# qcraftai/gedepth

Measured on AMD Instinct MI355X. Metric: training img/s (whole node), KITTI-shaped 352x1120 synthetic batches, higher is better.
Workload: dtype bf16; 1 GPU; depthformer_swint_v: DepthFormer-SwinT + GEDepth-Vanilla, 352x1120, 8 img/GPU, full train step; global_batch=8, parallelism=dp1, allreduce_dtype=fp32, layout=nhwc, window_attention=bf16 mfma, params=53516992, hip_graph=off

## Files before the change

gedepth_amd/csrc/common.h:

```cpp
#pragma once
#include <hip/hip_runtime.h>
#include <stdint.h>
#include "../../include/gedepth_hip.h"

#define GE_WAVE 64

#define GE_LAUNCH_CHECK()                         \
  do {                                            \
    hipError_t e__ = hipGetLastError();           \
    if (e__ != hipSuccess) return (int)e__;       \
  } while (0)

typedef uint16_t bf16_t;

__device__ __forceinline__ float bf2f(bf16_t h) { return __uint_as_float(((uint32_t)h) << 16); }
typedef __bf16 ge_bf16x8 __attribute__((ext_vector_type(8)));
typedef __bf16 ge_bf16x4 __attribute__((ext_vector_type(4)));
typedef __bf16 ge_bf16x2 __attribute__((ext_vector_type(2)));
typedef float ge_f32x16 __attribute__((ext_vector_type(16)));
typedef unsigned int ge_u32x4 __attribute__((ext_vector_type(4)));
typedef short ge_s16x2 __attribute__((ext_vector_type(2)));
#define GE_LDS(T, p) ((__attribute__((address_space(3))) T*)(p))

__device__ __forceinline__ bf16_t f2bf_hw(float f) { return __builtin_bit_cast(bf16_t, (__bf16)f); }
__device__ __forceinline__ uint32_t ge_pack_bf16x2(float lo, float hi) {
  ge_bf16x2 v = {(__bf16)lo, (__bf16)hi};
  return __builtin_bit_cast(uint32_t, v);
}
__device__ __forceinline__ bf16_t f2bf(float f) {
#ifndef GE_SW_BF16
  return f2bf_hw(f);
#endif
  uint32_t u = __float_as_uint(f);
  if ((u & 0x7fffffffu) > 0x7f800000u) return (bf16_t)((u >> 16) | 0x40u);
  u += 0x7fffu + ((u >> 16) & 1u);
  return (bf16_t)(u >> 16);
}

template <typename T> struct Io;
template <> struct Io<float> {
  static __device__ __forceinline__ float ld(const float* p) { return *p; }
  static __device__ __forceinline__ void st(float* p, float v) { *p = v; }
  static __device__ __forceinline__ float rt(float v) { return v; }
};
template <> struct Io<bf16_t> {
  static __device__ __forceinline__ float ld(const bf16_t* p) { return bf2f(*p); }
  static __device__ __forceinline__ void st(bf16_t* p, float v) { *p = f2bf(v); }
  static __device__ __forceinline__ float rt(float v) { return bf2f(f2bf(v)); }
};

template <typename T, int N> struct Vec;
template <> struct Vec<float, 4> {
  static __device__ __forceinline__ void ld(const float* p, float v[4]) { const float4 t = *(const float4*)p; v[0] = t.x; v[1] = t.y; v[2] = t.z; v[3] = t.w; }
  static __device__ __forceinline__ void st(float* p, const float v[4]) { *(float4*)p = make_float4(v[0], v[1], v[2], v[3]); }
};
template <> struct Vec<float, 8> {
  static __device__ __forceinline__ void ld(const float* p, float v[8]) { Vec<float, 4>::ld(p, v); Vec<float, 4>::ld(p + 4, v + 4); }
  static __device__ __forceinline__ void st(float* p, const float v[8]) { Vec<float, 4>::st(p, v); Vec<float, 4>::st(p + 4, v + 4); }
};
// ... 149 lines not shown
```

gedepth_amd/csrc/nhwc.hip:

```cpp
#include "common.h"
#include "../../include/gedepth_neck.h"

#define NH_MAXLANES 256

#define NH_MAXBLOCKS 1024
template <int K, int VN>
__device__ __forceinline__ void nh_col_commit(float (&acc)[K][VN], float* __restrict__ partial, int C, int lpr, int rpi, int c0) {
  __shared__ float sm[K][NH_MAXLANES][VN];
  const int t = threadIdx.x, rs = t / lpr;
#pragma unroll
  for (int k = 0; k < K; ++k)
#pragma unroll
    for (int v = 0; v < VN; ++v) sm[k][t][v] = acc[k][v];
  __syncthreads();
  int span = 1;
  while (span < rpi) span <<= 1;
  for (int stride = span >> 1; stride > 0; stride >>= 1) {
    if (rs < stride && rs + stride < rpi) {
#pragma unroll
      for (int k = 0; k < K; ++k)
#pragma unroll
        for (int v = 0; v < VN; ++v) sm[k][t][v] += sm[k][t + stride * lpr][v];
    }
    __syncthreads();
// ... 682 lines not shown
static int colsum_launch(const void* x, long R, int C, float* out, void* ws, int accumulate, hipStream_t s) {
  constexpr int VN = V8<T>::N;
  if (C % VN || !nh_aligned(x)) return GE_ERR_UNSUPPORTED;
  const int lanes = C / VN;
  int lpr = lanes < NH_MAXLANES ? lanes : NH_MAXLANES;
  while (lanes % lpr) --lpr;
  const int rpi = NH_MAXLANES / lpr, chunks = lanes / lpr;
  unsigned gx = nh_grid_rows(R, rpi);
  if (chunks > 1) gx = (gx + chunks - 1) / chunks;
  if (!gx) gx = 1;
  colsum_k<T><<<dim3(gx, chunks), 256, 0, s>>>((const T*)x, nh_partials(ws, C, 1), C, R, lpr, rpi);
  GE_LAUNCH_CHECK();
  nh_reduce_launch_f32(ws, C, gx, out, accumulate, s);
  GE_LAUNCH_CHECK();
  return GE_OK;
}
extern "C" int ge_colsum(const void* x, long R, int C, float* out, void* workspace, int accumulate, int dtype, void* stream) {
  if (!x || !out || !workspace || R < 0 || C <= 0) return GE_ERR_BAD_ARG;
  if (dtype == GE_F32) return colsum_launch<float>(x, R, C, out, workspace, accumulate, ge_stream(stream));
  if (dtype == GE_BF16) return colsum_launch<bf16_t>(x, R, C, out, workspace, accumulate, ge_stream(stream));
  return GE_ERR_UNSUPPORTED;
}

struct NhLevels { int s[GE_NECK_MAX_LEVELS + 1]; };
struct NhParts { const void* p[GE_NECK_MAX_LEVELS]; long pitch[GE_NECK_MAX_LEVELS]; long col[GE_NECK_MAX_LEVELS]; };
static bool nh_levels(const long* starts, int n, long N, NhLevels& lv, long& longest) {
  if (!starts || n < 1 || n > GE_NECK_MAX_LEVELS || N <= 0 || N > NH_WALK_MAX_ROWS || starts[0] != 0 || starts[n] != N) return false;
  longest = 0;
  for (int l = 0; l <= GE_NECK_MAX_LEVELS; ++l) lv.s[l] = (int)N;
  for (int l = 0; l < n; ++l) {
    if (starts[l + 1] < starts[l]) return false;
    lv.s[l] = (int)starts[l];
    if (starts[l + 1] - starts[l] > longest) longest = starts[l + 1] - starts[l];
  }
  return true;
}

template <typename T>
__global__ void __launch_bounds__(256) add_rows_levels_k(const T* __restrict__ x, const float* __restrict__ pos, const float* __restrict__ emb,
                                                         T* __restrict__ out, int B, long N, int C, NhLevels lv, int lpr, int rpi) {
  constexpr int VN = V8<T>::N;
  const int t = threadIdx.x, lane = t % lpr, rs = t / lpr, level = blockIdx.y;
  const int start = lv.s[level], nl = lv.s[level + 1] - start;
  if (rs >= rpi || nl <= 0) return;
  const int c0 = lane * VN;
  float e[VN];
// ... 247 lines not shown
```

gedepth_amd/depth/models/necks/hahi.py:

```python
import os

import torch
import torch.nn as nn
import torch.nn.functional as F

from .... import kernels as K
from .... import neck_kernels as NK
from ....kernels import add_rows, concat_tokens_map, ms_deform_attn_raw, residual_dropout, tokens_from_map
from ....mmrt import bricks
from ....mmrt.bricks import BaseModule, ConvModule, build_positional_encoding, xavier_init
from ..builder import ATTENTION, NECKS


@ATTENTION.register_module()
class MultiScaleDeformableAttention(BaseModule):

    def __init__(self, embed_dims=256, num_heads=8, num_levels=4, num_points=4, im2col_step=64, dropout=0.1,
                 batch_first=False, norm_cfg=None, init_cfg=None):
        super().__init__(init_cfg)
        if embed_dims % num_heads != 0:
            raise ValueError(f'embed_dims must be divisible by num_heads, but got {embed_dims} and {num_heads}')
        if embed_dims // num_heads != 64:
            raise NotImplementedError('the HIP sampling kernel is specialised for 64 channels per head')
        self.norm_cfg, self.batch_first = norm_cfg, batch_first
        self.dropout = nn.Dropout(dropout)
        self.im2col_step = im2col_step
        self.embed_dims, self.num_levels, self.num_heads, self.num_points = embed_dims, num_levels, num_heads, num_points
        self.sampling_offsets = nn.Linear(embed_dims, num_heads * num_levels * num_points * 2)
        self.attention_weights = nn.Linear(embed_dims, num_heads * num_levels * num_points)
        self.value_proj = bricks.Linear(embed_dims, embed_dims)
        self.output_proj = bricks.Linear(embed_dims, embed_dims)
        self.init_weights()

    def init_weights(self):
        bricks.constant_init(self.sampling_offsets, 0.)
        self.sampling_offsets.bias.data = bricks.msda_offset_bias(self.num_heads, self.num_levels, self.num_points)
        bricks.constant_init(self.attention_weights, val=0., bias=0.)
        xavier_init(self.value_proj, distribution='uniform', bias=0.)
        xavier_init(self.output_proj, distribution='uniform', bias=0.)
        self._is_init = True

    def _attend(self, query, value, reference_points, spatial_shapes, key_padding_mask=None, query_shapes=None, query_order=None):
        bs, num_query, _ = query.shape
        num_value = value.shape[1]
        if torch.is_tensor(spatial_shapes):
            spatial_shapes = [(int(h), int(w)) for h, w in spatial_shapes.tolist()]
        assert sum(h * w for h, w in spatial_shapes) == num_value
        if reference_points.shape[-1] != 2:
            raise ValueError('only 2-d reference points are used on the GEDepth path')
        value = self.value_proj(value)
        if key_padding_mask is not None:
            value = value.masked_fill(key_padding_mask[..., None], 0.0)
        value = value.view(bs, num_value, self.num_heads, -1)
        nH, L, P = self.num_heads, self.num_levels, self.num_points
        w = torch.cat((self.sampling_offsets.weight, self.attention_weights.weight), 0)
        b = torch.cat((self.sampling_offsets.bias, self.attention_weights.bias), 0)
        raw = bricks.linear_tokens(query, w, b)
        if raw.dtype != value.dtype:
            raw = raw.to(value.dtype)
        ref = reference_points.expand(bs, num_query, L, 2)
        if query_order is not None and 'msda_mm' not in K.DISABLED and K.msda_mm_supported(value, raw, spatial_shapes, nH, L, P):
            out = K.ms_deform_attn_mm(value, raw, ref, spatial_shapes, query_order, nH, L, P)
        elif K.msda_self_split_ok(value, raw, spatial_shapes, query_shapes, nH, L, P):
            out = K.ms_deform_attn_self_split(value, raw, ref, spatial_shapes, nH, L, P)
        else:
            out = ms_deform_attn_raw(value, raw, ref, spatial_shapes, query_shapes, nH, L, P)
        return self.output_proj(out)

    def forward(self, query, key=None, value=None, identity=None, query_pos=None, key_padding_mask=None,
                reference_points=None, spatial_shapes=None, level_start_index=None, query_shapes=None, query_order=None, **kwargs):
        if value is None:
            value = query
        if identity is None:
            identity = query
        if query_pos is not None:
            if query_pos.dim() == 3 and query_pos.shape[0] == 1 and query_pos.dtype == torch.float32 and query.dim() == 3 and self.batch_first:
                query = add_rows(query, query_pos[0])
            else:
                query = query + query_pos.to(query.dtype)
        if not self.batch_first:
            query, value = query.permute(1, 0, 2), value.permute(1, 0, 2)
        out = self._attend(query, value, reference_points, spatial_shapes, key_padding_mask, query_shapes, query_order)
        if not self.batch_first:
            out = out.permute(1, 0, 2)
        if self.training and self.dropout.p > 0 and out.is_cuda and out.dim() == 3 and self.batch_first:
            return residual_dropout(identity, out, self.dropout.p)
        return self.dropout(out) + identity

    def forward_map(self, fmap, pos_map, value, reference_points, spatial_shapes, concat_with, query_order=None, query=None):
        if query is None:
            query = tokens_from_map(fmap, pos_map)
        out = self._attend(query, value, reference_points, spatial_shapes, query_shapes=[tuple(fmap.shape[2:])], query_order=query_order)
        p = self.dropout.p if self.training else 0.0
        return concat_tokens_map(out, concat_with, identity=fmap, tokens_first=True, p_drop=p)


@NECKS.register_module()
class HAHIHeteroNeck(BaseModule):

    def __init__(self, in_channels, out_channels, embedding_dim, scales=[1, 1, 1, 1],
                 norm_cfg=dict(type='BN', requires_grad=True), act_cfg=dict(type='ReLU', inplace=True),
                 cross_att=True, self_att=True, constrain=False, positional_encoding=None, num_points=8):
        super().__init__()
        assert isinstance(in_channels, list)
        assert all(s == 1 for s in scales), 'GEDepth configs use scale 1 at every level'
        self.cross_att, self.self_att, self.constrain = cross_att, self_att, constrain
        self.in_channels, self.out_channels, self.scales = in_channels, out_channels, scales
        self.num_outs = len(scales)
        self.embedding_dim = E = embedding_dim
        cm = dict(norm_cfg=norm_cfg, act_cfg=act_cfg)
        self.lateral_convs = nn.ModuleList(ConvModule(i, o, kernel_size=1, **cm) for i, o in zip(in_channels, out_channels))
        self.trans_proj = nn.ModuleList(ConvModule(o, E, kernel_size=1, **cm) for o in out_channels[1:])
        self.trans_fusion = nn.ModuleList(ConvModule(o + E, o, kernel_size=3, padding=1, stride=1, **cm)
                                          for o in out_channels[1:])
        self.conv_proj = nn.Sequential(ConvModule(in_channels[0], E, kernel_size=1, **cm))
        self.conv_fusion = nn.Sequential(ConvModule(in_channels[0] + E, out_channels[0], kernel_size=3, padding=1,
                                                    stride=1, **cm))
# ... 134 lines not shown
```

gedepth_amd/hip.py:

```python
import ctypes
import os
import re

import torch

_HERE = os.path.dirname(os.path.abspath(__file__))
LIB_PATH = os.environ.get('GE_LIB') or os.path.join(_HERE, 'csrc', 'libgedepth_hip.so')
HEADERS = {'SIGNATURES': 'gedepth_hip.h', 'EVAL_SIGNATURES': 'gedepth_eval.h', 'DDAD_SIGNATURES': 'gedepth_ddad.h',
           'CLOUD_SIGNATURES': 'gedepth_cloud.h', 'GROUND_SIGNATURES': 'gedepth_ground.h'}
EXTRA_HEADERS = {'BATCH_SIGNATURES': 'gedepth_batch.h'}
SCENE_HEADERS = {'SCENE_SIGNATURES': 'gedepth_scene.h'}
STRATA_HEADERS = {'STRATA_SIGNATURES': 'gedepth_strata.h'}
NECK_HEADERS = {'NECK_SIGNATURES': 'gedepth_neck.h'}
GE_F32, GE_BF16 = 0, 1
GE_COLORIZE_VMIN_DATA, GE_COLORIZE_VMAX_DATA, GE_COLORIZE_EQUAL = 1, 2, 4

_SCALARS = {'int': ctypes.c_int, 'long': ctypes.c_long, 'float': ctypes.c_float, 'double': ctypes.c_double, 'size_t': ctypes.c_size_t,
            'uint64_t': ctypes.c_ulonglong, 'unsigned long long': ctypes.c_ulonglong}
_DECL = re.compile(r'\b(int|size_t)\s+(ge_\w+)\s*\(([^()]*)\)\s*;')


def parse_header(text):
    text = re.sub(r'/\*.*?\*/|//[^\n]*', ' ', text, flags=re.S)
    sigs = {}
    for res, name, params in _DECL.findall(text):
        args = []
        for p in ([] if params.strip() == 'void' else params.split(',')):
            if '*' in p:
                args.append(ctypes.c_void_p)
                continue
            ctype = ' '.join(w for w in p.split()[:-1] if w != 'const')
            if ctype not in _SCALARS:
                raise TypeError(f'{name}: parameter "{" ".join(p.split())}" has a type the ctypes binding does not map')
            args.append(_SCALARS[ctype])
        sigs[name] = (_SCALARS[res], args)
    stray = set(re.findall(r'\b(ge_\w+)\s*\(', text)) - set(sigs)
    if stray:
        raise TypeError(f'cannot parse the declaration of {", ".join(sorted(stray))}')
    return sigs


for _table, _header in {**HEADERS, **EXTRA_HEADERS, **SCENE_HEADERS, **STRATA_HEADERS, **NECK_HEADERS}.items():
    with open(os.path.join(os.path.dirname(_HERE), 'include', _header)) as _fh:
        globals()[_table] = parse_header(_fh.read())

_lib = None


class HipLibraryError(RuntimeError):
    pass


def lib():
    global _lib
    if _lib is None:
        if not os.path.isfile(LIB_PATH):
            raise HipLibraryError(
                f'{LIB_PATH} is missing: the gfx950 HIP kernels are not built. '
                f'Run gedepth_amd/csrc/build.sh (hipcc --offload-arch=gfx950). There is no CPU/eager fallback.')
        handle = ctypes.CDLL(LIB_PATH)
        for table in (*HEADERS, *EXTRA_HEADERS, *SCENE_HEADERS, *STRATA_HEADERS, *NECK_HEADERS):
            for name, (res, args) in globals()[table].items():
                fn = getattr(handle, name)
                fn.restype, fn.argtypes = res, args
        _lib = handle
        if os.environ.get('GE_MSDA_MODE'):
            handle.ge_msda_mode(int(os.environ['GE_MSDA_MODE']))
    return _lib


def is_built():
    return os.path.isfile(LIB_PATH)


def check(code, what):
    if code != 0:
        raise RuntimeError(f'{what} failed with code {code} '
                           f'({"bad argument" if code == 10001 else "unsupported" if code == 10002 else "hipError_t"})')


def call(name, *args):
    code = getattr(_lib or lib(), name)(*args)
    if code:
        check(code, name)
# ... 26 lines not shown
```

gedepth_amd/kernels.py:

```python
import ctypes
import os

import torch

from . import hip

_f32 = torch.float32


def _c(t):
    return t if t.is_contiguous() else t.contiguous()


class _Profiler:

    def __init__(self):
        self.on, self.records, self.stage_bytes = False, {}, {}

    def enable(self):
        self.on, self.records, self.stage_bytes = True, {}, {}
        hip.lib().ge_msda_bwd_timing(1)

    def disable(self):
        self.on = False
# ... 256 lines not shown
    nbytes = (value.numel() * _es(value) + (loc.numel() + attw.numel()) * 4 + d_raw.numel() * es + d_out.numel() * _es(d_out)
              + (0 if d_value is None else d_value.numel() * 4))
    _launch(f'msda_bwd_raw[B{B} Nq{Nq} Nv{Nv} {_tag(value)}{" lw" if d_value is None else ""}]', nbytes, 'ge_msda_bwd_raw', hip.ptr(value), lv.ptr,
            grid.ptr, grid.n, hip.ptr(loc), hip.ptr(attw), hip.ptr(d_out), hip.ptr(d_value), base, ld, base + nH * L * P * 2 * es, ld, hip.ptr(d_ref),
            hip.ptr(ws), ws_bytes, B, Nv, Nq, nH, L, P, hip.dtype_code(value), hip.stream())
    return d_raw, d_ref


def _bwd_value_records(raw, raw_ref, d_out, d_value, lv, nH, L, P, level_mask=15):
    B, Nq, _ = raw.shape
    Nv = d_value.shape[1]
    n_off = nH * L * P * 2
    ws_bytes = int(hip.lib().ge_msda_bwd_workspace(lv.ptr, B, Nv, Nq, nH, L, P))
    ws = torch.empty(ws_bytes, device=raw.device, dtype=torch.uint8)
    frac = bin(level_mask).count('1') / 4
    if PROFILER.on:
        PROFILER.add_stage_bytes((0, B * Nq * n_off * 2, 0, raw.numel() * 2, int(frac * d_out.numel() * 2) + d_value.numel() * 4))
    _launch(f'msda_bwd_value_raw[B{B} Nq{Nq} Nv{Nv}{"" if level_mask == 15 else f" levels {level_mask:04b}"}]',
            B * Nq * n_off * 2 + raw.numel() * 2 + d_out.numel() * 2 + d_value.numel() * 4, 'ge_msda_bwd_value_raw_levels', lv.ptr,
            *raw_ref, hip.ptr(d_out), hip.ptr(d_value), hip.ptr(ws), ws_bytes, level_mask, B, Nv, Nq, nH, L, P,
            hip.dtype_code(d_out), hip.stream())


class _MSDeformAttnRaw(torch.autograd.Function):

    @staticmethod
    def forward(ctx, value, raw, ref, spatial_shapes, query_shapes, nH, L, P):
        value, raw = _c(value), _c(raw)
        assert value.shape[3] == 64 and raw.shape[2] == nH * L * P * 3 and raw.dtype == value.dtype
        lv, grid = _levels(spatial_shapes), _query_grid(query_shapes, raw.shape[1])
        out, loc, attw, ref = _window_fwd_raw(value, raw, ref, lv, grid, nH, L, P)
        ctx.value_from_raw = (value.dtype == torch.bfloat16 and L == 4 and P == 8 and 'msda_value_raw' not in DISABLED
                              and max(max(hw) for hw in lv.hw) <= 8191)
        if ctx.value_from_raw:
            ctx.save_for_backward(value, loc, attw, raw, ref)
        else:
            ctx.save_for_backward(value, loc, attw)
        ctx.meta = (lv, grid, nH, L, P)
        ctx.last_loc = loc
        return out

    @staticmethod
    def backward(ctx, d_out):
        value, loc, attw = ctx.saved_tensors[:3]
        split = ctx.value_from_raw
        lv, grid, nH, L, P = ctx.meta
        d_out = _c(d_out.to(value.dtype))
        d_value = torch.zeros(value.shape, device=value.device, dtype=_f32)
        d_raw, d_ref = _window_bwd_raw(value, loc, attw, d_out, lv, grid, None if split else d_value, ctx.needs_input_grad[2])
        if PROFILER.on:
            lw_b = value.numel() * _es(value) + (loc.numel() + attw.numel()) * 4 + d_raw.numel() * _es(d_raw) + d_out.numel() * _es(d_out)
            la_b = (loc.numel() + attw.numel()) * 4
            PROFILER.add_stage_bytes((lw_b, 0, 0, 0, 0) if split else (lw_b, la_b, 0, la_b, d_out.numel() * _es(d_out) + d_value.numel() * 4))
        if split:
            raw, ref = ctx.saved_tensors[3:]
            _bwd_value_records(raw, _raw_ref(raw, ref, nH, L, P)[0], d_out, d_value, lv, nH, L, P)
        return d_value.to(value.dtype), d_raw, d_ref, None, None, None, None, None


def ms_deform_attn_raw(value, raw, reference_points, spatial_shapes, query_shapes, num_heads, num_levels, num_points):
    B, Nv = value.shape[:2]
    Nq = raw.shape[1]
    fused = ('msda_raw' not in DISABLED and query_shapes is not None and MSDA_BINNED_BACKWARD and value.is_cuda and raw.dtype == value.dtype
             and value.dtype in (_f32, torch.bfloat16))
    if fused:
        lv, grid = _levels(spatial_shapes), _query_grid(query_shapes, Nq)
        fused = bool(hip.lib().ge_msda_raw_supported(lv.ptr, grid.ptr, grid.n, B, Nv, Nq, num_heads, num_levels, num_points))
        fused = fused and int(hip.lib().ge_msda_bwd_workspace(lv.ptr, B, Nv, Nq, num_heads, num_levels, num_points)) > 0
    if not fused:
        loc, attw = msda_prepare(raw, reference_points, spatial_shapes, num_heads, num_levels, num_points)
        return ms_deform_attn(value, spatial_shapes, loc, attw, query_shapes)
    return _MSDeformAttnRaw.apply(value, raw, reference_points, spatial_shapes, query_shapes, int(num_heads), int(num_levels), int(num_points))


_TILE_ORDER_CACHE = {}


def msda_tile_order(query_shapes, device, th=4, tw=8):
    key = (tuple(tuple(int(v) for v in hw) for hw in query_shapes), str(device), th, tw)
    if key not in _TILE_ORDER_CACHE:
        parts, start = [], 0
        for h, w in key[0]:
            idx = torch.arange(h * w, dtype=torch.int64).view(h, w)
            ph, pw = (-h) % th, (-w) % tw
            idx = torch.nn.functional.pad(idx, (0, pw, 0, ph), value=-1)
            hh, ww = idx.shape
            t = idx.view(hh // th, th, ww // tw, tw).permute(0, 2, 1, 3).reshape(-1)
            parts.append(t[t >= 0] + start)
            start += h * w
        _TILE_ORDER_CACHE[key] = torch.cat(parts).to(torch.int32).to(device)
    return _TILE_ORDER_CACHE[key]


# ... 68 lines not shown
                self.mm_mask = 15 if t_mm < (1.1 if on else 0.9) * t_rec else 0
                self.last = dict(rows=rows, passes=passes, mm_ms=round(t_mm * 1e-6, 3), records_ms=round(t_rec * 1e-6, 3),
                                 per_level=[dict(rows=int(host[2 + 2 * l]), passes=int(host[3 + 2 * l])) for l in range(4)])


_MM_VALUE_CHOICE = {}


def _mm_value_choice(key, mm_ok, rec_ok):
    c = _MM_VALUE_CHOICE.get(key)
    if c is None:
        c = _MM_VALUE_CHOICE[key] = _MMValueChoice()
    c.update()
    mask = c.mm_mask if c.forced is None else c.forced
    mask = 0 if not mm_ok else 15 if not rec_ok else mask
    return c, mask


class _MSDeformAttnMM(torch.autograd.Function):

    @staticmethod
    def forward(ctx, value, raw, ref, order, spatial_shapes, nH, L, P):
        lv = _levels(spatial_shapes)
        out = msda_fwd_mm(value, raw, ref, lv, order, want_loc=False, nH=nH, L=L, P=P)
        ctx.save_for_backward(value, raw, ref, order)
        ctx.meta = (lv, nH, L, P)
        return out

    @staticmethod
    def backward(ctx, d_out):
        value, raw, ref, order = ctx.saved_tensors
        lv, nH, L, P = ctx.meta
        value, raw = _c(value), _c(raw)
        B, Nv, _, D = value.shape
        _, Nq, ld = raw.shape
        d_out = _c(d_out.to(value.dtype))
        raw_ref, ref = _raw_ref(raw, ref, nH, L, P)
        lib = hip.lib()
        d_raw = torch.empty(B, Nq, ld, device=value.device, dtype=raw.dtype)
        dbase = hip.ptr(d_raw)
        nb_lw = value.numel() * 2 + raw.numel() * 2 + d_raw.numel() * 2 + d_out.numel() * 2
        want_dv = ctx.needs_input_grad[0]
        use_vs = (want_dv and os.environ.get('GE_MSDA_VALUE') == 'vs' and B * Nq * ld * 2 < 2 ** 32 and B * Nq * nH * D * 2 < 2 ** 32
                  and 0 <= ref.stride(1) and Nq * ref.stride(1) * 4 < 2 ** 32)
        vs_ws_bytes = int(lib.ge_msda_bwd_vs_workspace(lv.ptr, B, Nv, Nq, nH, L, P)) if use_vs else 0
        mm_ws_bytes = int(lib.ge_msda_bwd_mm_workspace(B, Nq, nH, L)) if (want_dv and 'msda_value_mm' not in DISABLED) else 0
        if vs_ws_bytes:
            mm_ws_bytes = vs_ws_bytes
        mm_ws = torch.empty(mm_ws_bytes, device=value.device, dtype=torch.uint8) if mm_ws_bytes else None
        _launch(f'msda_mm_bwd_lw_k[B{B} Nq{Nq} Nv{Nv}]', nb_lw, 'ge_msda_bwd_lw_mm', hip.ptr(value), lv.ptr, *raw_ref, hip.ptr(order), hip.ptr(d_out),
                dbase, ld, dbase + nH * L * P * 2 * 2, ld, hip.ptr(mm_ws), B, Nv, Nq, nH, L, P, hip.dtype_code(value), hip.stream())
        d_ref = None
        if ctx.needs_input_grad[2]:
            d_ref = torch.empty(B, Nq, L, 2, device=value.device, dtype=_f32)
            hip.call('ge_msda_dref', dbase, ld, lv.ptr, hip.ptr(d_ref), B * Nq, nH, L, P, hip.dtype_code(value), hip.stream())
        d_value = None
        if want_dv:
            d_value = torch.zeros(B, Nv, nH, D, device=value.device, dtype=_f32)
            if vs_ws_bytes:
                _launch(f'msda_mm_bwd_vs_k[B{B} Nq{Nq} Nv{Nv}]', raw.numel() * 2 + d_out.numel() * 2 + d_value.numel() * 4, 'ge_msda_bwd_value_vs', lv.ptr,
                        *raw_ref, hip.ptr(order), hip.ptr(d_out), hip.ptr(d_value), hip.ptr(mm_ws), mm_ws_bytes, B, Nv, Nq, nH, L, P,
                        hip.dtype_code(value), hip.stream())
                return d_value.to(value.dtype), d_raw, d_ref, None, None, None, None, None
            rec_ws_bytes = int(lib.ge_msda_bwd_workspace(lv.ptr, B, Nv, Nq, nH, L, P))
            choice, mm_mask = _mm_value_choice((B, Nq, Nv, nH, lv.hw, str(value.device)), mm_ws is not None, rec_ws_bytes > 0)
            rec_mask = 15 & ~mm_mask

            def value_mm(dv, mask):
                return (lv.ptr, *raw_ref, hip.ptr(order), hip.ptr(d_out), hip.ptr(dv), hip.ptr(mm_ws), mm_ws_bytes, mask, B, Nv, Nq, nH, L, P,
                        hip.dtype_code(value), hip.stream())
            if mm_mask:
                lv_rows = sum(h * w for l, (h, w) in enumerate(lv.hw) if (mm_mask >> l) & 1)
                _launch(f'msda_mm_bwd_v_k[B{B} Nq{Nq} Nv{Nv} levels {mm_mask:04b}]',
                        bin(mm_mask).count('1') * (raw.numel() // 2 + d_out.numel() * 2 // 4) + B * lv_rows * nH * D * 4, 'ge_msda_bwd_value_mm',
                        *value_mm(d_value, mm_mask))
            elif mm_ws is not None and choice.wants_stats():
                hip.call('ge_msda_bwd_value_mm', *value_mm(None, 0))
            if rec_mask:
                if rec_ws_bytes <= 0:
                    raise RuntimeError('ms_deform_attn_mm backward: neither the MFMA d_value kernel nor the binned path covers this geometry')
                _bwd_value_records(raw, raw_ref, d_out, d_value, lv, nH, L, P, rec_mask)
            if mm_ws is not None:
                choice.observe(mm_ws, int(lib.ge_msda_bwd_mm_stats_offset(B, Nq, nH, L)), B * Nq * nH)
            d_value = d_value.to(value.dtype)
        return d_value, d_raw, d_ref, None, None, None, None, None


def msda_mm_supported(value, raw, spatial_shapes, nH, L, P):
    if not (value.is_cuda and value.dtype == torch.bfloat16 and raw.dtype == torch.bfloat16 and value.shape[-1] == 64):
        return False
    B, Nv = value.shape[:2]
    return bool(hip.lib().ge_msda_mm_supported(_levels(spatial_shapes).ptr, B, Nv, raw.shape[1], nH, L, P, hip.GE_BF16))


def ms_deform_attn_mm(value, raw, reference_points, spatial_shapes, order, num_heads=8, num_levels=4, num_points=8):
    return _MSDeformAttnMM.apply(value, raw, reference_points, order, spatial_shapes, int(num_heads), int(num_levels), int(num_points))


class _MSDeformAttnSelfSplit(torch.autograd.Function):

    @staticmethod
    def forward(ctx, value, raw, ref, spatial_shapes, n_fine, order_fine, nH, L, P):
        value, raw = _c(value), _c(raw)
        B, Nv, _, D = value.shape
        _, Nq, ld = raw.shape
        assert D == 64 and ld == nH * L * P * 3 and raw.dtype == value.dtype == torch.bfloat16 and 0 < n_fine < Nq
        raw_ref, ref = _raw_ref(raw, ref, nH, L, P)
        lv = _levels(spatial_shapes)
        out = torch.empty(B, Nq, nH * D, device=value.device, dtype=value.dtype)
        nc = Nq - n_fine
        _launch(f'msda_mm_fwd_k[B{B} Nq{n_fine}/{Nq} Nv{Nv}]', value.numel() * 2 + B * n_fine * (ld + nH * D) * 2, 'ge_msda_fwd_mm_part',
                hip.ptr(value, name='value'), lv.ptr, *raw_ref, hip.ptr(order_fine), hip.ptr(out), B, Nv, n_fine, Nq, nH, L, P, hip.GE_BF16, hip.stream())
        coarse_shapes = []
        acc = 0
        for hw in lv.hw:
            acc += hw[0] * hw[1]
            if acc > n_fine:
                coarse_shapes.append(hw)
        assert sum(h * w for h, w in coarse_shapes) == nc, 'n_fine must end on a level boundary'
        grid = _query_grid(coarse_shapes, nc)
        out[:, n_fine:], loc, attw, _ = _window_fwd_raw(value, raw[:, n_fine:].contiguous(), ref[:, n_fine:], lv, grid, nH, L, P)
        ctx.save_for_backward(value, raw, ref, order_fine, loc, attw)
        ctx.meta = (lv, grid, n_fine, nH, L, P)
        return out

    @staticmethod
    def backward(ctx, d_out):
        value, raw, ref, order_fine, loc, attw = ctx.saved_tensors
        lv, grid, n_fine, nH, L, P = ctx.meta
        B, Nv, _, D = value.shape
        _, Nq, ld = raw.shape
        d_out = _c(d_out.to(value.dtype))
        raw_ref, _ = _raw_ref(raw, ref, nH, L, P)
        d_raw = torch.empty(B, Nq, ld, device=value.device, dtype=raw.dtype)
        dbase = hip.ptr(d_raw)
        _launch(f'msda_mm_bwd_lw_k[B{B} Nq{n_fine}/{Nq} Nv{Nv}]', value.numel() * 2 + B * n_fine * (2 * ld + nH * D) * 2, 'ge_msda_bwd_lw_mm_part',
                hip.ptr(value), lv.ptr, *raw_ref, hip.ptr(order_fine), hip.ptr(d_out), dbase, ld, dbase + nH * L * P * 2 * 2, ld, B, Nv, n_fine, Nq,
                nH, L, P, hip.GE_BF16, hip.stream())
        d_raw[:, n_fine:], _ = _window_bwd_raw(value, loc, attw, d_out[:, n_fine:].contiguous(), lv, grid)
        d_value = None
        if ctx.needs_input_grad[0]:
            d_value = torch.zeros(B, Nv, nH, D, device=value.device, dtype=_f32)
            _bwd_value_records(raw, raw_ref, d_out, d_value, lv, nH, L, P)
            d_value = d_value.to(value.dtype)
        return d_value, d_raw, None, None, None, None, None, None, None


def msda_self_split_ok(value, raw, spatial_shapes, query_shapes, nH, L, P):
    if 'msda_self_split' in DISABLED or 'msda_mm' in DISABLED or 'msda_raw' in DISABLED or 'msda_value_raw' in DISABLED or not MSDA_BINNED_BACKWARD:
        return False
    lv = _levels(spatial_shapes)
    shapes = lv.hw
    if query_shapes is None or _levels(query_shapes).hw != shapes or len(shapes) < 2 or L != 4 or P != 8:
        return False
    if not (value.is_cuda and value.dtype == torch.bfloat16 and raw.dtype == torch.bfloat16 and value.shape[-1] == 64 and max(max(hw) for hw in shapes) <= 8191):
        return False
    B, Nv = value.shape[:2]
    Nq = raw.shape[1]
    n_fine = shapes[0][0] * shapes[0][1]
    if Nq != Nv or not msda_mm_supported(value, raw, lv, nH, L, P):
        return False
    lib = hip.lib()
    grid = _query_grid(shapes[1:], Nq - n_fine)
    return (bool(lib.ge_msda_raw_supported(lv.ptr, grid.ptr, grid.n, B, Nv, Nq - n_fine, nH, L, P)) and int(lib.ge_msda_bwd_workspace(lv.ptr, B, Nv, Nq - n_fine, nH, L, P)) > 0
            and int(lib.ge_msda_bwd_workspace(lv.ptr, B, Nv, Nq, nH, L, P)) > 0)


# ... 1280 lines not shown
```

gedepth_amd/mmrt/bricks.py:

```python
import math
import warnings

import torch
import torch.nn as nn
import torch.nn.functional as F

from .registry import Registry, build_from_cfg

MODELS = Registry('model')
ATTENTION = Registry('attention')
POSITIONAL_ENCODING = Registry('position encoding')
DROPOUT_LAYERS = Registry('drop out layers')


def constant_init(module, val, bias=0):
    if hasattr(module, 'weight') and module.weight is not None:
        nn.init.constant_(module.weight, val)
    if hasattr(module, 'bias') and module.bias is not None:
        nn.init.constant_(module.bias, bias)


def xavier_init(module, gain=1, bias=0, distribution='normal'):
    assert distribution in ['uniform', 'normal']
    if hasattr(module, 'weight') and module.weight is not None:
# ... 133 lines not shown

    @staticmethod
    def backward(ctx, dy):
        xc, wc = ctx.saved_tensors
        splits, x_dtype, w_dtype, b_dtype = ctx.meta
        K = xc.numel() // xc.shape[-1]
        with torch.autocast('cuda', enabled=False):
            dy2 = dy.to(wc.dtype).reshape(K, -1)
            x2 = xc.reshape(K, -1)
            dx = dw = db = None
            if not dy2.is_contiguous():
                dy2 = dy2.contiguous()
            if ctx.needs_input_grad[0]:
                dx = _linear_dx(dy2, wc).reshape(xc.shape).to(x_dtype)
            if ctx.needs_input_grad[1]:
                if splits:
                    M, N = dy2.shape[1], x2.shape[1]
                    part = torch.bmm(dy2.view(splits, K // splits, M).transpose(1, 2), x2.view(splits, K // splits, N))
                    dw = _sum_partials(part, ctx.weight_ref, w_dtype)
                else:
                    dw = _plain_dw(dy2, x2, ctx.weight_ref, w_dtype)
            if b_dtype is not None and ctx.needs_input_grad[2]:
                if dy2.shape[1] % (4 if dy2.dtype == torch.float32 else 8) == 0:
                    from .. import kernels
                    db = kernels.colsum(dy2 if dy2.is_contiguous() else dy2.contiguous()).to(b_dtype)
                else:
                    db = dy2.sum(0, dtype=torch.float32).to(b_dtype)
        return dx, dw, db, None


class _LinearBiasGelu(torch.autograd.Function):

    @staticmethod
    def forward(ctx, x, weight, bias, splits):
        from .. import kernels
        dt = torch.get_autocast_dtype('cuda') if torch.is_autocast_enabled() else x.dtype
        with torch.autocast('cuda', enabled=False):
            from .optim import lowp
            xc, wc = x.to(dt), lowp(weight, dt)
            y0 = _linear_fwd(xc, wc, weight, bias, dt)
            g = kernels.bias_gelu_fwd(y0, None)
        ctx.save_for_backward(xc, wc, y0)
        ctx.meta = (splits, x.dtype, weight.dtype, bias.dtype)
        ctx.weight_ref = weight if isinstance(weight, nn.Parameter) else None
        return g

    @staticmethod
    def backward(ctx, dg):
# ... 238 lines not shown
    keep_prob = 1 - drop_prob
    shape = (x.shape[0],) + (1,) * (x.ndim - 1)
    random_tensor = keep_prob + torch.rand(shape, dtype=x.dtype, device=x.device)
    return x.div(keep_prob) * random_tensor.floor()


@DROPOUT_LAYERS.register_module()
class DropPath(nn.Module):

    def __init__(self, drop_prob=0.1):
        super().__init__()
        self.drop_prob = drop_prob

    def forward(self, x):
        return drop_path(x, self.drop_prob, self.training)

    def residual(self, identity, branch):
        if (not identity.is_cuda or self.drop_prob == 0. or not self.training or identity.shape != branch.shape
                or (identity.dtype, branch.dtype) not in _RESIDUAL_DTYPES):
            if identity.is_cuda and self.training and self.drop_prob > 0.:
                from .. import kernels
                kernels.note_fallback('DropPath.residual', f'{identity.dtype}+{branch.dtype} {tuple(identity.shape)} vs {tuple(branch.shape)}')
            return identity + self(branch)
        from .. import kernels
        return kernels.residual_drop_path(identity, branch, _DROP_PATH_BANK.scale(self, branch.shape[0], branch.dtype, branch.device))


class _DropPathBank:

    def __init__(self):
        self.layers, self.rows, self.used, self.key, self.keep = [], None, [], None, None
        self.probs = None
        self.seed, self.offset = None, 0

    def scale(self, layer, batch, dtype, device):
        idx = getattr(layer, '_bank_index', None)
        key = (batch, device)
        if idx is None or idx >= len(self.layers) or self.layers[idx]() is not layer:
            import weakref
            self.layers = [r for r in self.layers if r() is not None]
            for i, r in enumerate(self.layers):
                r()._bank_index = i
            idx = layer._bank_index = len(self.layers)
            self.layers.append(weakref.ref(layer))
            self.rows = self.keep = None
        gen = torch.cuda.default_generators[device.index if device.index is not None else torch.cuda.current_device()] if device.type == 'cuda' else None
        capturing = gen is not None and torch.cuda.is_current_stream_capturing()
        reseeded = gen is not None and not capturing and (gen.initial_seed(), gen.get_offset() >= self.offset) != (self.seed, True)
# ... 87 lines not shown
```

Baseline: 178.3 img/s.

## Fuse bias-gradient column sums into upstream backward elementwise kernels

```diff
diff --git a/gedepth_amd/csrc/common.h b/gedepth_amd/csrc/common.h
--- a/gedepth_amd/csrc/common.h
+++ b/gedepth_amd/csrc/common.h
@@ -35,6 +35,11 @@
   if ((u & 0x7fffffffu) > 0x7f800000u) return (bf16_t)((u >> 16) | 0x40u);
   u += 0x7fffu + ((u >> 16) & 1u);
   return (bf16_t)(u >> 16);
+}
+
+__device__ __forceinline__ float ge_mul_rounded(float a, float b) {
+#pragma clang fp contract(off)
+  return a * b;
 }
 
 template <typename T> struct Io;
diff --git a/gedepth_amd/csrc/nhwc.hip b/gedepth_amd/csrc/nhwc.hip
--- a/gedepth_amd/csrc/nhwc.hip
+++ b/gedepth_amd/csrc/nhwc.hip
@@ -1,5 +1,6 @@
 #include "common.h"
 #include "../../include/gedepth_neck.h"
+#include "../../include/gedepth_grad.h"
 
 #define NH_MAXLANES 256
 
@@ -728,6 +729,155 @@
   return GE_ERR_UNSUPPORTED;
 }
 
+struct NhColGeom { int lpr, rpi, chunks; unsigned gx; };
+template <int VN>
+static bool nh_colsum_geom(long R, int C, NhColGeom& g) {
+  if (C <= 0 || C % VN) return false;
+  const int lanes = C / VN;
+  g.lpr = lanes < NH_MAXLANES ? lanes : NH_MAXLANES;
+  while (lanes % g.lpr) --g.lpr;
+  g.rpi = NH_MAXLANES / g.lpr; g.chunks = lanes / g.lpr;
+  g.gx = nh_grid_rows(R, g.rpi);
+  if (g.chunks > 1) g.gx = (g.gx + g.chunks - 1) / g.chunks;
+  if (!g.gx) g.gx = 1;
+  return true;
+}
+template <typename TI, typename TO>
+__global__ void __launch_bounds__(256) scale_rows_colsum_k(const TI* __restrict__ x, const float* __restrict__ scale, TO* __restrict__ out,
+                                                           float* __restrict__ ws, int C, long R, int rps, int lpr, int rpi) {
+  constexpr int VN = V8<TO>::N;
+  const int t = threadIdx.x, lane = t % lpr, rs = t / lpr;
+  const int c0 = (blockIdx.y * lpr + lane) * VN;
+  float acc[1][VN];
+#pragma unroll
+  for (int v = 0; v < VN; ++v) acc[0][v] = 0.f;
+  const long r0 = (long)blockIdx.x * rpi + rs, step = (long)gridDim.x * rpi;
+  if (rs < rpi && r0 < R) {
+    NhWalk w((unsigned)r0, (unsigned)step, rps);
+    for (long r = r0; r < R; r += step, w.next()) {
+      const float sc = scale[w.img];
+      float v[VN];
+      Vec<TI, VN>::ld(x + r * C + c0, v);
+#pragma unroll
+      for (int k = 0; k < VN; ++k) {
+        v[k] = Io<TO>::rt(ge_mul_rounded(v[k], sc));
+        acc[0][k] += v[k];
+      }
+      Vec<TO, VN>::st(out + r * C + c0, v);
+    }
+  }
+  nh_col_commit<1, VN>(acc, ws, C, lpr, rpi, c0);
+}
+template <typename T>
+__global__ void __launch_bounds__(256) slice_rows_drop_colsum_k(const T* __restrict__ d_out, T* __restrict__ d_a, float* __restrict__ ws, long R,
+                                                                int Ca, int Co, int off_a, float p, float inv_keep, uint64_t seed0,
+                                                                const unsigned long long* __restrict__ salt, int lpr, int rpi) {
+  const uint64_t seed = ge_salted(seed0, salt);
+  const uint32_t thr = ge_drop_threshold(p);
+  constexpr int VN = V8<T>::N;
+  const int t = threadIdx.x, lane = t % lpr, rs = t / lpr;
+  const int c0 = (blockIdx.y * lpr + lane) * VN;
+  float acc[1][VN];
+#pragma unroll
+  for (int v = 0; v < VN; ++v) acc[0][v] = 0.f;
+  if (rs < rpi)
+    for (long r = (long)blockIdx.x * rpi + rs; r < R; r += (long)gridDim.x * rpi) {
+      float v[VN];
+      V8<T>::ld(d_out + r * Co + off_a + c0, v);
+      if (p > 0.f) {
+#pragma unroll
+        for (int k0 = 0; k0 < VN; k0 += 4) {
+          float sc[4];
+          ge_drop_scale4(seed, (uint64_t)(r * Ca + c0 + k0) >> 2, thr, inv_keep, sc);
+#pragma unroll
+          for (int e = 0; e < 4; ++e) v[k0 + e] = ge_mul_rounded(v[k0 + e], sc[e]);
+        }
+      }
+#pragma unroll
+      for (int k = 0; k < VN; ++k) {
+        v[k] = Io<T>::rt(v[k]);
+        acc[0][k] += v[k];
+      }
+      V8<T>::st(d_a + r * Ca + c0, v);
+    }
+  nh_col_commit<1, VN>(acc, ws, Ca, lpr, rpi, c0);
+}
+__global__ void __launch_bounds__(256) cast_rows_colsum_k(const float* __restrict__ x, bf16_t* __restrict__ out, float* __restrict__ ws, int C, long R,
+                                                          int lpr, int rpi) {
+  constexpr int VN = 8;
+  const int t = threadIdx.x, lane = t % lpr, rs = t / lpr;
+  const int c0 = (blockIdx.y * lpr + lane) * VN;
+  float acc[1][VN];
+#pragma unroll
+  for (int v = 0; v < VN; ++v) acc[0][v] = 0.f;
+  if (rs < rpi)
+    for (long r = (long)blockIdx.x * rpi + rs; r < R; r += (long)gridDim.x * rpi) {
+      float v[VN];
+      Vec<float, VN>::ld(x + r * C + c0, v);
+#pragma unroll
+      for (int k = 0; k < VN; ++k) {
+        v[k] = v[k] != v[k] ? __uint_as_float(0x7fc00000u) : bf2f(f2bf_hw(v[k]));
+        acc[0][k] += v[k];
+      }
+      Vec<bf16_t, VN>::st(out + r * C + c0, v);
+    }
+  nh_col_commit<1, VN>(acc, ws, C, lpr, rpi, c0);
+}
+
+template <typename TI, typename TO>
+static int scale_rows_colsum_launch(const void* x, const float* scale, void* out, float* d_bias, void* ws, long R, long rps, int C, hipStream_t s) {
+  NhColGeom g;
+  if (!nh_colsum_geom<V8<TO>::N>(R, C, g) || !nh_aligned(x, out)) return GE_ERR_UNSUPPORTED;
+  scale_rows_colsum_k<TI, TO><<<dim3(g.gx, g.chunks), 256, 0, s>>>((const TI*)x, scale, (TO*)out, nh_partials(ws, C, 1), C, R, (int)rps, g.lpr, g.rpi);
+  GE_LAUNCH_CHECK();
+  nh_reduce_launch_f32(ws, C, g.gx, d_bias, 0, s);
+  GE_LAUNCH_CHECK();
+  return GE_OK;
+}
+extern "C" int ge_scale_rows_colsum(const void* x, int x_dtype, const float* scale, void* out, int out_dtype, float* d_bias, void* workspace,
+                                    long rows, long rows_per_sample, int C, void* stream) {
+  if (!x || !scale || !out || !d_bias || !workspace || rows < 0 || rows >= (1L << 31) || C <= 0) return GE_ERR_BAD_ARG;
+  if (rows_per_sample <= 0 || rows_per_sample > NH_WALK_MAX_ROWS || rows % rows_per_sample) return GE_ERR_BAD_ARG;
+  hipStream_t s = ge_stream(stream);
+  if (x_dtype == GE_F32 && out_dtype == GE_BF16) return scale_rows_colsum_launch<float, bf16_t>(x, scale, out, d_bias, workspace, rows, rows_per_sample, C, s);
+  if (x_dtype == GE_BF16 && out_dtype == GE_BF16) return scale_rows_colsum_launch<bf16_t, bf16_t>(x, scale, out, d_bias, workspace, rows, rows_per_sample, C, s);
+  if (x_dtype == GE_F32 && out_dtype == GE_F32) return scale_rows_colsum_launch<float, float>(x, scale, out, d_bias, workspace, rows, rows_per_sample, C, s);
+  return GE_ERR_UNSUPPORTED;
+}
+template <typename T>
+static int slice_rows_drop_colsum_launch(const void* d_out, void* d_a, float* d_bias, void* ws, long R, int Ca, int Co, int off_a, float p,
+                                         unsigned long long seed, hipStream_t s) {
+  NhColGeom g;
+  if (!nh_colsum_geom<V8<T>::N>(R, Ca, g) || Co % V8<T>::N || off_a % V8<T>::N || !nh_aligned(d_out, d_a)) return GE_ERR_UNSUPPORTED;
+  const float inv_keep = p > 0.f ? 1.f / (1.f - p) : 1.f;
+  slice_rows_drop_colsum_k<T><<<dim3(g.gx, g.chunks), 256, 0, s>>>((const T*)d_out, (T*)d_a, nh_partials(ws, Ca, 1), R, Ca, Co, off_a, p, inv_keep, seed,
+                                                                   ge_rng_salt_get(), g.lpr, g.rpi);
+  GE_LAUNCH_CHECK();
+  nh_reduce_launch_f32(ws, Ca, g.gx, d_bias, 0, s);
+  GE_LAUNCH_CHECK();
+  return GE_OK;
+}
+extern "C" int ge_slice_rows_drop_colsum(const void* d_out, void* d_a, float* d_bias, void* workspace, long rows, int Ca, int Co, int off_a,
+                                         float p_drop, unsigned long long seed, int dtype, void* stream) {
+  if (!d_out || !d_a || !d_bias || !workspace || rows < 0 || rows >= (1L << 31) || Ca <= 0 || Co < Ca || off_a < 0 || off_a + Ca > Co || p_drop < 0.f ||
+      p_drop >= 1.f)
+    return GE_ERR_BAD_ARG;
+  if (dtype == GE_F32) return slice_rows_drop_colsum_launch<float>(d_out, d_a, d_bias, workspace, rows, Ca, Co, off_a, p_drop, seed, ge_stream(stream));
+  if (dtype == GE_BF16) return slice_rows_drop_colsum_launch<bf16_t>(d_out, d_a, d_bias, workspace, rows, Ca, Co, off_a, p_drop, seed, ge_stream(stream));
+  return GE_ERR_UNSUPPORTED;
+}
+extern "C" int ge_cast_rows_colsum(const float* x, void* out, float* d_bias, void* workspace, long rows, int C, void* stream) {
+  if (!x || !out || !d_bias || !workspace || rows < 0 || rows >= (1L << 31) || C <= 0) return GE_ERR_BAD_ARG;
+  NhColGeom g;
+  if (!nh_colsum_geom<8>(rows, C, g) || !nh_aligned(x, out)) return GE_ERR_UNSUPPORTED;
+  hipStream_t s = ge_stream(stream);
+  cast_rows_colsum_k<<<dim3(g.gx, g.chunks), 256, 0, s>>>(x, (bf16_t*)out, nh_partials(workspace, C, 1), C, rows, g.lpr, g.rpi);
+  GE_LAUNCH_CHECK();
+  nh_reduce_launch_f32(workspace, C, g.gx, d_bias, 0, s);
+  GE_LAUNCH_CHECK();
+  return GE_OK;
+}
+
 struct NhLevels { int s[GE_NECK_MAX_LEVELS + 1]; };
 struct NhParts { const void* p[GE_NECK_MAX_LEVELS]; long pitch[GE_NECK_MAX_LEVELS]; long col[GE_NECK_MAX_LEVELS]; };
 static bool nh_levels(const long* starts, int n, long N, NhLevels& lv, long& longest) {
diff --git a/gedepth_amd/depth/models/necks/hahi.py b/gedepth_amd/depth/models/necks/hahi.py
--- a/gedepth_amd/depth/models/necks/hahi.py
+++ b/gedepth_amd/depth/models/necks/hahi.py
@@ -4,9 +4,10 @@
 import torch.nn as nn
 import torch.nn.functional as F
 
+from .... import grad_kernels as GK
 from .... import kernels as K
 from .... import neck_kernels as NK
-from ....kernels import add_rows, concat_tokens_map, ms_deform_attn_raw, residual_dropout, tokens_from_map
+from ....kernels import add_rows, concat_tokens_map, ms_deform_attn_raw, tokens_from_map
 from ....mmrt import bricks
 from ....mmrt.bricks import BaseModule, ConvModule, build_positional_encoding, xavier_init
 from ..builder import ATTENTION, NECKS
@@ -51,6 +52,7 @@
         value = self.value_proj(value)
         if key_padding_mask is not None:
             value = value.masked_fill(key_padding_mask[..., None], 0.0)
+        value_tokens = value if GK.enabled() and value.dtype == torch.bfloat16 and value.is_contiguous() else None
         value = value.view(bs, num_value, self.num_heads, -1)
         nH, L, P = self.num_heads, self.num_levels, self.num_points
         w = torch.cat((self.sampling_offsets.weight, self.attention_weights.weight), 0)
@@ -60,11 +62,11 @@
             raw = raw.to(value.dtype)
         ref = reference_points.expand(bs, num_query, L, 2)
         if query_order is not None and 'msda_mm' not in K.DISABLED and K.msda_mm_supported(value, raw, spatial_shapes, nH, L, P):
-            out = K.ms_deform_attn_mm(value, raw, ref, spatial_shapes, query_order, nH, L, P)
+            out = K.ms_deform_attn_mm(value if value_tokens is None else value_tokens, raw, ref, spatial_shapes, query_order, nH, L, P)
         elif K.msda_self_split_ok(value, raw, spatial_shapes, query_shapes, nH, L, P):
-            out = K.ms_deform_attn_self_split(value, raw, ref, spatial_shapes, nH, L, P)
-        else:
-            out = ms_deform_attn_raw(value, raw, ref, spatial_shapes, query_shapes, nH, L, P)
+            out = K.ms_deform_attn_self_split(value if value_tokens is None else value_tokens, raw, ref, spatial_shapes, nH, L, P)
+        else:
+            out = ms_deform_attn_raw(value if value_tokens is None else value_tokens, raw, ref, spatial_shapes, query_shapes, nH, L, P)
         return self.output_proj(out)
 
     def forward(self, query, key=None, value=None, identity=None, query_pos=None, key_padding_mask=None,
@@ -84,7 +86,7 @@
         if not self.batch_first:
             out = out.permute(1, 0, 2)
         if self.training and self.dropout.p > 0 and out.is_cuda and out.dim() == 3 and self.batch_first:
-            return residual_dropout(identity, out, self.dropout.p)
+            return GK.residual_dropout(identity, out, self.dropout.p)
         return self.dropout(out) + identity
 
     def forward_map(self, fmap, pos_map, value, reference_points, spatial_shapes, concat_with, query_order=None, query=None):
@@ -92,7 +94,7 @@
             query = tokens_from_map(fmap, pos_map)
         out = self._attend(query, value, reference_points, spatial_shapes, query_shapes=[tuple(fmap.shape[2:])], query_order=query_order)
         p = self.dropout.p if self.training else 0.0
-        return concat_tokens_map(out, concat_with, identity=fmap, tokens_first=True, p_drop=p)
+        return GK.concat_tokens_map(out, concat_with, identity=fmap, tokens_first=True, p_drop=p)
 
 
 @NECKS.register_module()
diff --git a/gedepth_amd/grad_kernels.py b/gedepth_amd/grad_kernels.py
--- /dev/null
+++ b/gedepth_amd/grad_kernels.py
@@ -0,0 +1,138 @@
+import torch
+
+from . import hip
+from . import kernels as K
+from .kernels import _c, _cl, _es, _f32, _launch, _raw_ptr, _tag
+
+handed_over = 0
+recomputed = 0
+_ATTR = '_ge_dy_colsum'
+_WS = {}
+
+
+def enabled():
+    return 'dy_colsum' not in K.DISABLED
+
+
+def _workspace(device, C):
+    key = (device, hip.stream(), C)
+    ws = _WS.get(key)
+    if ws is None:
+        ws = _WS[key] = torch.empty(int(hip.lib().ge_nhwc_workspace(C, 1)), device=device, dtype=torch.uint8)
+    return ws
+
+
+def attach(dy, d_bias):
+    setattr(dy, _ATTR, (d_bias, dy.data_ptr(), tuple(dy.shape), dy.dtype, dy._version))
+    return dy
+
+
+def take(dy, dtype):
+    ent = getattr(dy, _ATTR, None)
+    if ent is None:
+        return None
+    delattr(dy, _ATTR)
+    d_bias, ptr, shape, dt, version = ent
+    if (dy.data_ptr(), tuple(dy.shape), dy.dtype, dy._version) != (ptr, shape, dt, version):
+        return None
+    if dt != dtype or not dy.is_contiguous() or dy.dim() < 2 or d_bias.numel() != dy.shape[-1]:
+        return None
+    return d_bias
+
+
+def bias_grad(dy, dy2):
+    global handed_over, recomputed
+    d_bias = take(dy, dy2.dtype) if enabled() else None
+    if d_bias is not None:
+        handed_over += 1
+        return d_bias
+    recomputed += 1
+    return K.colsum(dy2 if dy2.is_contiguous() else dy2.contiguous())
+
+
+class _ResidualDropPath(K._ResidualDropPath):
+
+    @staticmethod
+    def backward(ctx, dy):
+        scale, = ctx.saved_tensors
+        dy = _c(dy)
+        B, N, C = dy.shape
+        d_branch = torch.empty(dy.shape, device=dy.device, dtype=ctx.branch_dtype)
+        d_bias = torch.empty(C, device=dy.device, dtype=_f32)
+        _launch(f'scale_rows_colsum[{B}x{N}x{C} {_tag(dy)}->{_tag(d_branch)}]', dy.numel() * _es(dy) + d_branch.numel() * _es(d_branch),
+                'ge_scale_rows_colsum', hip.ptr(dy), hip.dtype_code(dy), hip.ptr(scale), hip.ptr(d_branch), hip.dtype_code(d_branch), hip.ptr(d_bias),
+                hip.ptr(_workspace(dy.device, C)), B * N, N, C, hip.stream())
+        return dy, attach(d_branch, d_bias), None
+
+
+def drop_path_ok(identity, branch):
+    return (enabled() and branch.dim() == 3 and branch.dtype == torch.bfloat16 and branch.shape[2] % 8 == 0 and branch.numel() > 0
+            and identity.dtype in (_f32, torch.bfloat16) and 0 < branch.shape[1] <= 1 << 30 and branch.shape[0] * branch.shape[1] < 1 << 31)
+
+
+def residual_drop_path(identity, branch, scale):
+    return _ResidualDropPath.apply(identity, branch, scale)
+
+
+def _slice_rows_drop_colsum(d_out, d_tok, B, N, C, Co, off, p, seed):
+    d_bias = torch.empty(C, device=d_out.device, dtype=_f32)
+    _launch(f'slice_rows_drop_colsum[{B}x{N}x{C} {_tag(d_out)}]', 2 * d_tok.numel() * _es(d_out), 'ge_slice_rows_drop_colsum', _raw_ptr(d_out, 'd_out'),
+            hip.ptr(d_tok), hip.ptr(d_bias), hip.ptr(_workspace(d_out.device, C)), B * N, C, Co, off, p, seed, hip.dtype_code(d_out), hip.stream())
+    return attach(d_tok, d_bias)
+
+
+class _ResidualDropout(K._ResidualDropout):
+
+    @staticmethod
+    def backward(ctx, d_out):
+        B, N, C, p, seed, id_dtype = ctx.meta
+        d_out = _c(d_out)
+        d_tok = _slice_rows_drop_colsum(d_out, torch.empty_like(d_out), B, N, C, C, 0, p, seed)
+        return d_tok, d_out.to(id_dtype), None, None
+
+
+def residual_dropout(identity, tokens, p, seed=None):
+    vn = 8 if tokens.dtype == torch.bfloat16 else 4
+    if not (enabled() and tokens.is_cuda and tokens.dim() == 3 and tokens.dtype in (_f32, torch.bfloat16) and tokens.shape[2] % vn == 0
+            and identity.shape == tokens.shape and identity.dtype == tokens.dtype and 0.0 < p < 1.0 and 0 < tokens.shape[0] * tokens.shape[1] < 1 << 31):
+        return K.residual_dropout(identity, tokens, p, seed)
+    if seed is None:
+        seed = int(torch.randint(0, 2 ** 62, (1,)).item())
+    return _ResidualDropout.apply(tokens, identity, float(p), int(seed))
+
+
+class _ConcatRows(K._ConcatRows):
+
+    @staticmethod
+    def backward(ctx, d_out):
+        B, N, C, Cm, tokens_first, p, seed, has_id = ctx.meta
+        d_out = _cl(d_out)
+        t0, m0 = (0, C) if tokens_first else (Cm, 0)
+        d_tok = _slice_rows_drop_colsum(d_out, torch.empty(B, N, C, device=d_out.device, dtype=d_out.dtype), B, N, C, C + Cm, t0, p, seed)
+        return d_tok, d_out[:, m0:m0 + Cm], (d_out[:, t0:t0 + C] if has_id else None), None, None, None
+
+
+def concat_tokens_map(tokens, fmap, identity=None, tokens_first=True, p_drop=0.0, seed=None):
+    p_drop = float(p_drop)
+    vn = 8 if tokens.dtype == torch.bfloat16 else 4
+    if not (enabled() and p_drop > 0.0 and K._cl_ok(fmap) and tokens.dim() == 3 and tokens.shape[2] % vn == 0 and tokens.is_cuda
+            and tokens.dtype == fmap.dtype and tokens.stride(2) == 1 and tokens.stride(1) == tokens.shape[2] and tokens.stride(0) % vn == 0
+            and fmap.shape[1] % vn == 0 and 0 < tokens.shape[0] * tokens.shape[1] < 1 << 31):
+        return K.concat_tokens_map(tokens, fmap, identity, tokens_first, p_drop, seed)
+    if seed is None:
+        seed = int(torch.randint(0, 2 ** 62, (1,)).item())
+    return _ConcatRows.apply(tokens, fmap, identity, bool(tokens_first), p_drop, int(seed))
+
+
+def cast_rows(x, shape=None):
+    shape = tuple(x.shape if shape is None else shape)
+    C = shape[-1] if shape else 0
+    if not (enabled() and x.is_cuda and x.dtype == _f32 and x.is_contiguous() and len(shape) >= 2 and C > 0 and C % 8 == 0 and x.data_ptr() % 16 == 0
+            and 0 < x.numel() // C < 1 << 31):
+        return x.to(torch.bfloat16).view(shape)
+    R = x.numel() // C
+    out = torch.empty(shape, device=x.device, dtype=torch.bfloat16)
+    d_bias = torch.empty(C, device=x.device, dtype=_f32)
+    _launch(f'cast_rows_colsum[{R}x{C}]', x.numel() * 6, 'ge_cast_rows_colsum', hip.ptr(x), hip.ptr(out), hip.ptr(d_bias),
+            hip.ptr(_workspace(x.device, C)), R, C, hip.stream())
+    return attach(out, d_bias)
diff --git a/gedepth_amd/hip.py b/gedepth_amd/hip.py
--- a/gedepth_amd/hip.py
+++ b/gedepth_amd/hip.py
@@ -12,6 +12,7 @@
 SCENE_HEADERS = {'SCENE_SIGNATURES': 'gedepth_scene.h'}
 STRATA_HEADERS = {'STRATA_SIGNATURES': 'gedepth_strata.h'}
 NECK_HEADERS = {'NECK_SIGNATURES': 'gedepth_neck.h'}
+GRAD_HEADERS = {'GRAD_SIGNATURES': 'gedepth_grad.h'}
 GE_F32, GE_BF16 = 0, 1
 GE_COLORIZE_VMIN_DATA, GE_COLORIZE_VMAX_DATA, GE_COLORIZE_EQUAL = 1, 2, 4
 
@@ -40,7 +41,7 @@
     return sigs
 
 
-for _table, _header in {**HEADERS, **EXTRA_HEADERS, **SCENE_HEADERS, **STRATA_HEADERS, **NECK_HEADERS}.items():
+for _table, _header in {**HEADERS, **EXTRA_HEADERS, **SCENE_HEADERS, **STRATA_HEADERS, **NECK_HEADERS, **GRAD_HEADERS}.items():
     with open(os.path.join(os.path.dirname(_HERE), 'include', _header)) as _fh:
         globals()[_table] = parse_header(_fh.read())
 
@@ -59,7 +60,7 @@
                 f'{LIB_PATH} is missing: the gfx950 HIP kernels are not built. '
                 f'Run gedepth_amd/csrc/build.sh (hipcc --offload-arch=gfx950). There is no CPU/eager fallback.')
         handle = ctypes.CDLL(LIB_PATH)
-        for table in (*HEADERS, *EXTRA_HEADERS, *SCENE_HEADERS, *STRATA_HEADERS, *NECK_HEADERS):
+        for table in (*HEADERS, *EXTRA_HEADERS, *SCENE_HEADERS, *STRATA_HEADERS, *NECK_HEADERS, *GRAD_HEADERS):
             for name, (res, args) in globals()[table].items():
                 fn = getattr(handle, name)
                 fn.restype, fn.argtypes = res, args
diff --git a/gedepth_amd/kernels.py b/gedepth_amd/kernels.py
--- a/gedepth_amd/kernels.py
+++ b/gedepth_amd/kernels.py
@@ -302,11 +302,23 @@
             hip.dtype_code(d_out), hip.stream())
 
 
+def _value_heads(ctx, value, nH):
+    ctx.value_shape = tuple(value.shape)
+    return value.view(value.shape[0], value.shape[1], nH, -1) if value.dim() == 3 else value
+
+
+def _d_value_out(ctx, d_value, dtype):
+    if dtype == torch.bfloat16:
+        from . import grad_kernels
+        return grad_kernels.cast_rows(d_value, ctx.value_shape)
+    return d_value.to(dtype).view(ctx.value_shape)
+
+
 class _MSDeformAttnRaw(torch.autograd.Function):
 
     @staticmethod
     def forward(ctx, value, raw, ref, spatial_shapes, query_shapes, nH, L, P):
-        value, raw = _c(value), _c(raw)
+        value, raw = _c(_value_heads(ctx, value, nH)), _c(raw)
         assert value.shape[3] == 64 and raw.shape[2] == nH * L * P * 3 and raw.dtype == value.dtype
         lv, grid = _levels(spatial_shapes), _query_grid(query_shapes, raw.shape[1])
         out, loc, attw, ref = _window_fwd_raw(value, raw, ref, lv, grid, nH, L, P)
@@ -335,7 +347,7 @@
         if split:
             raw, ref = ctx.saved_tensors[3:]
             _bwd_value_records(raw, _raw_ref(raw, ref, nH, L, P)[0], d_out, d_value, lv, nH, L, P)
-        return d_value.to(value.dtype), d_raw, d_ref, None, None, None, None, None
+        return _d_value_out(ctx, d_value, value.dtype), d_raw, d_ref, None, None, None, None, None
 
 
 def ms_deform_attn_raw(value, raw, reference_points, spatial_shapes, query_shapes, num_heads, num_levels, num_points):
@@ -349,6 +361,8 @@
         fused = fused and int(hip.lib().ge_msda_bwd_workspace(lv.ptr, B, Nv, Nq, num_heads, num_levels, num_points)) > 0
     if not fused:
         loc, attw = msda_prepare(raw, reference_points, spatial_shapes, num_heads, num_levels, num_points)
+        if value.dim() == 3:
+            value = value.view(B, Nv, num_heads, -1)
         return ms_deform_attn(value, spatial_shapes, loc, attw, query_shapes)
     return _MSDeformAttnRaw.apply(value, raw, reference_points, spatial_shapes, query_shapes, int(num_heads), int(num_levels), int(num_points))
 
@@ -463,6 +477,7 @@
     @staticmethod
     def forward(ctx, value, raw, ref, order, spatial_shapes, nH, L, P):
         lv = _levels(spatial_shapes)
+        value = _value_heads(ctx, value, nH)
         out = msda_fwd_mm(value, raw, ref, lv, order, want_loc=False, nH=nH, L=L, P=P)
         ctx.save_for_backward(value, raw, ref, order)
         ctx.meta = (lv, nH, L, P)
@@ -502,7 +517,7 @@
                 _launch(f'msda_mm_bwd_vs_k[B{B} Nq{Nq} Nv{Nv}]', raw.numel() * 2 + d_out.numel() * 2 + d_value.numel() * 4, 'ge_msda_bwd_value_vs', lv.ptr,
                         *raw_ref, hip.ptr(order), hip.ptr(d_out), hip.ptr(d_value), hip.ptr(mm_ws), mm_ws_bytes, B, Nv, Nq, nH, L, P,
                         hip.dtype_code(value), hip.stream())
-                return d_value.to(value.dtype), d_raw, d_ref, None, None, None, None, None
+                return _d_value_out(ctx, d_value, value.dtype), d_raw, d_ref, None, None, None, None, None
             rec_ws_bytes = int(lib.ge_msda_bwd_workspace(lv.ptr, B, Nv, Nq, nH, L, P))
             choice, mm_mask = _mm_value_choice((B, Nq, Nv, nH, lv.hw, str(value.device)), mm_ws is not None, rec_ws_bytes > 0)
             rec_mask = 15 & ~mm_mask
@@ -523,7 +538,7 @@
                 _bwd_value_records(raw, raw_ref, d_out, d_value, lv, nH, L, P, rec_mask)
             if mm_ws is not None:
                 choice.observe(mm_ws, int(lib.ge_msda_bwd_mm_stats_offset(B, Nq, nH, L)), B * Nq * nH)
-            d_value = d_value.to(value.dtype)
+            d_value = _d_value_out(ctx, d_value, value.dtype)
         return d_value, d_raw, d_ref, None, None, None, None, None
 
 
@@ -542,7 +557,7 @@
 
     @staticmethod
     def forward(ctx, value, raw, ref, spatial_shapes, n_fine, order_fine, nH, L, P):
-        value, raw = _c(value), _c(raw)
+        value, raw = _c(_value_heads(ctx, value, nH)), _c(raw)
         B, Nv, _, D = value.shape
         _, Nq, ld = raw.shape
         assert D == 64 and ld == nH * L * P * 3 and raw.dtype == value.dtype == torch.bfloat16 and 0 < n_fine < Nq
@@ -583,7 +598,7 @@
         if ctx.needs_input_grad[0]:
             d_value = torch.zeros(B, Nv, nH, D, device=value.device, dtype=_f32)
             _bwd_value_records(raw, raw_ref, d_out, d_value, lv, nH, L, P)
-            d_value = d_value.to(value.dtype)
+            d_value = _d_value_out(ctx, d_value, value.dtype)
         return d_value, d_raw, None, None, None, None, None, None, None
 
 
diff --git a/gedepth_amd/mmrt/bricks.py b/gedepth_amd/mmrt/bricks.py
--- a/gedepth_amd/mmrt/bricks.py
+++ b/gedepth_amd/mmrt/bricks.py
@@ -179,8 +179,8 @@
                     dw = _plain_dw(dy2, x2, ctx.weight_ref, w_dtype)
             if b_dtype is not None and ctx.needs_input_grad[2]:
                 if dy2.shape[1] % (4 if dy2.dtype == torch.float32 else 8) == 0:
-                    from .. import kernels
-                    db = kernels.colsum(dy2 if dy2.is_contiguous() else dy2.contiguous()).to(b_dtype)
+                    from .. import grad_kernels
+                    db = grad_kernels.bias_grad(dy, dy2).to(b_dtype)
                 else:
                     db = dy2.sum(0, dtype=torch.float32).to(b_dtype)
         return dx, dw, db, None
@@ -465,8 +465,11 @@
                 from .. import kernels
                 kernels.note_fallback('DropPath.residual', f'{identity.dtype}+{branch.dtype} {tuple(identity.shape)} vs {tuple(branch.shape)}')
             return identity + self(branch)
-        from .. import kernels
-        return kernels.residual_drop_path(identity, branch, _DROP_PATH_BANK.scale(self, branch.shape[0], branch.dtype, branch.device))
+        from .. import grad_kernels, kernels
+        scale = _DROP_PATH_BANK.scale(self, branch.shape[0], branch.dtype, branch.device)
+        if grad_kernels.drop_path_ok(identity, branch):
+            return grad_kernels.residual_drop_path(identity, branch, scale)
+        return kernels.residual_drop_path(identity, branch, scale)
 
 
 class _DropPathBank:
diff --git a/include/gedepth_grad.h b/include/gedepth_grad.h
--- /dev/null
+++ b/include/gedepth_grad.h
@@ -0,0 +1,22 @@
+#ifndef GEDEPTH_GRAD_H
+#define GEDEPTH_GRAD_H
+
+#include <stddef.h>
+#include <stdint.h>
+
+#ifdef __cplusplus
+extern "C" {
+#endif
+
+int ge_scale_rows_colsum(const void* x, int x_dtype, const float* scale, void* out, int out_dtype, float* d_bias, void* workspace, long rows,
+                         long rows_per_sample, int C, void* stream);
+
+int ge_slice_rows_drop_colsum(const void* d_out, void* d_a, float* d_bias, void* workspace, long rows, int Ca, int Co, int off_a, float p_drop,
+                              unsigned long long seed, int dtype, void* stream);
+
+int ge_cast_rows_colsum(const float* x, void* out, float* d_bias, void* workspace, long rows, int C, void* stream);
+
+#ifdef __cplusplus
+}
+#endif
+#endif
```

After: 179.7 img/s, median of 6. Within noise of the previous version (+0.8%).
